# r-papso/carca-replication

Measured on AMD Instinct MI355X. Metric: scored users/sec (1+100 candidates), CARCA eval forward, higher is better.
Workload: dtype f32

## Files before the change

carca_replication_amd/_lib.py:

```python
from __future__ import annotations

import ctypes as C
import hashlib
import os
import shutil
import subprocess
import threading

_HERE = os.path.dirname(os.path.abspath(__file__))
_CSRC = os.path.join(_HERE, "csrc")
_INCLUDE = os.path.join(os.path.dirname(_HERE), "include")
LIB_PATH = os.path.join(_HERE, "libcarca_hip.so")
_STAMP = LIB_PATH + ".srchash"
SOURCES = ["api.hip", "gemm.hip", "gemm_wgrad.hip", "gemm_split.hip", "gemm_stream.hip", "wgrad_cu.hip", "decoders.hip", "batch_build.hip", "embed.hip", "sa_block.hip", "sa_eval.hip", "cross_score.hip", "cross_stream.hip", "loss_metrics.hip", "backward.hip", "block_bwd.hip", "row_chain.hip", "optim.hip", "recommend.hip", "rank.hip", "knn_catalogue.hip",
           "catalogue_xent.hip", "feat_dedup.hip", "sampled_xent.hip", "sampled_bce.hip", "similar_items.hip", "mmr_rerank.hip", "recommend_lists.hip", "explain_lists.hip"]
HEADERS = ["carca_common.h", "gemm_host.h", "attn_common.h", "gemm_epilogue.h", "cross_fold.h", "recommend_common.h", "catalogue_select.h",
           "catalogue_sweep.h", "xent_tile.h", "xent_stage.h", "row_stream.h", "group_select.h"]

MAX_SEGS = 4
MAX_GROUPS = 3
MAX_L = 64
MAX_PROFILE_L = 1024

_lock = threading.Lock()
# ... 299 lines not shown
    "carca_poll_errors": (_i, []),
    "carca_capture_scope": (_i, [_fp, C.POINTER(C.c_ulonglong)]),
    "carca_capture_bytes": (C.c_longlong, [C.c_ulonglong]),
    "carca_capture_release": (_i, [C.c_ulonglong]),
    "carca_release_stream_scratch": (_i, [_fp]),
    "carca_padded_dims": (_i, [_i, _i, C.POINTER(_i), C.POINTER(_i), C.POINTER(_i)]),
    "carca_attn_geometry_built": (_i, [_i, _i]),
    "carca_pack_weights": (_i, [C.POINTER(PackDesc), _i, _fp]),
    "carca_embed_fwd": (_i, [C.POINTER(RowSeg), _i, _i, _i, _i, _i, _fp, _fp, _fp, _fp, _fp, _fp, _fp, _i, _i, _fp]),
    "carca_gemm_rows": (_i, [C.POINTER(GemmDesc), _fp]),
    "carca_split_bytes": (C.c_longlong, [_i, _i, _i]),
    "carca_split_pack": (_i, [_fp, _i, _i, _i, _i, _fp, _fp]),
    "carca_split_bind": (_i, [_fp, _fp, _i, _i, _i]),
    "carca_split_launch_count": (C.c_longlong, []),
    "carca_gemm_rows_group": (_i, [C.POINTER(GemmDesc), _i, _fp]),
    "carca_gemm_wgrad": (_i, [C.POINTER(WgradDesc), _fp]),
    "carca_gemm_wgrad_group": (_i, [C.POINTER(WgradDesc), _i, _fp]),
    "carca_sa_block_fwd": (_i, [_fp, _i, _fp, _fp, _i, _i, _i, _i, _i, C.POINTER(SaWeights), _i, C.POINTER(SaSave),
                                C.POINTER(Dropout), _fp]),
    "carca_sa_block_eval": (_i, [_fp, _i, _fp, _fp, _i, _i, _i, _i, _i, C.POINTER(SaWeights), _i, _i, _fp]),
    "carca_cross_score_fwd": (_i, [_fp, _i, _fp, _fp, C.POINTER(TargetGroup), _i, _i, _i, _i, _i, _i,
                                   C.POINTER(CaWeights), _i, _i, C.POINTER(CaSave), C.POINTER(Dropout), _fp]),
    "carca_dropout_fwd": (_i, [_fp, _i, _i, _i, C.POINTER(Dropout), _fp, _fp]),
    "carca_mask_mul": (_i, [_fp, _i, _fp, _i, _f, _fp, _i, _i, _i, _i, _fp]),
    "carca_layernorm_bwd": (_i, [_fp, _i, _fp, _i, _fp, _i, _i, _fp, _i, _fp, _i, _i, _fp, _fp, _fp]),
    "carca_embed_scatter": (_i, [_fp, _i, _fp, _i, _i, _f, _fp, _fp]),
    "carca_colsum": (_i, [_fp, _i, _i, _i, _fp, _fp, _i, _fp, _fp]),
    "carca_sa_attn_bwd": (_i, [_fp, _fp, _fp, _fp, _i, _fp, _fp, _fp, _fp, _i, _i, _i, _i, _fp, _f, _fp]),
    "carca_cross_attn_bwd": (_i, [_fp, _fp, _fp, C.POINTER(CrossBwdGroup), _i, _fp, _fp, _fp, _fp, _i, _i, _i, _i, _i,
                                  _f, _fp]),
    "carca_unpack_grads": (_i, [C.POINTER(PackDesc), _i, _i, _fp]),
    "carca_forward": (_i, [C.POINTER(ForwardDesc), C.POINTER(_fp), _fp]),
    "carca_event_create": (_i, [C.POINTER(_fp)]),
    "carca_event_destroy": (_i, [_fp]),
    "carca_event_elapsed_ms": (_i, [_fp, _fp, C.POINTER(C.c_float)]),
    "carca_stream_wait_event": (_i, [_fp, _fp]),
    "carca_bce_fwd": (_i, [_fp, _fp, _fp, _i, _f, _fp, _fp, _fp, _fp, _fp]),
    "carca_rank_metrics": (_i, [_fp, _i, _i, _i, _fp, _fp, _fp, _fp]),
    "carca_eval_metrics": (_i, [_fp, _fp, _fp, _i, _i, _i, _f, _fp, _fp]),
    "carca_layernorm_fwd": (_i, [_fp, _i, _fp, _i, _i, _i, _fp, _fp, _fp]),
    "carca_dot_score_fwd": (_i, [_fp, _i, _fp, _i, _fp, _i, _i, _i, _i, _i, _i, _fp]),
    "carca_dot_score_bwd": (_i, [_fp, _i, _fp, _i, _fp, _fp, _fp, _i, _fp, _i, _i, _i, _i, _i, _i, _i, _fp]),
    "carca_slot_decay_scale": (_i, [_fp, _i, _fp, _i, _i, _i, _i, _f, _fp]),
    "carca_l2norm_fwd": (_i, [_fp, _i, _fp, _i, _i, _i, _fp]),
    "carca_l2norm_bwd": (_i, [_fp, _i, _fp, _i, _fp, _i, _i, _i, _fp]),
    "carca_add_positions": (_i, [_fp, _i, _fp, _fp, _i, _i, _i, _i, _fp]),
    "carca_mha_core": (_i, [_fp, _i, _fp, _fp, _i, _fp, _fp, _i, _i, _i, _i, _i, _i, _i, _fp, _i, _fp, _fp]),
    "carca_mha_core_bwd": (_i, [_fp, _i, _fp, _fp, _i, _fp, _fp, _i, _i, _i, _i, _i, _i, _i, _fp, _i, _fp, _fp, _fp, _fp,
                                _fp]),
    "carca_gemm_rows_log": (_i, [C.c_char_p, _i]),
    "carca_feat_dedup_rows_multiplied": (C.c_longlong, []),
    "carca_feat_dedup_rows_computed": (C.c_longlong, []),
    "carca_feat_dedup_rows_grouped": (C.c_longlong, []),
    "carca_feat_cache_arm": (_i, [C.POINTER(FeatCache)]),
    "carca_get_tuning": (_i, [_i]),
    "carca_mha_core_drop": (_i, [_fp, _i, _fp, _fp, _i, _fp, _fp, _i, _i, _i, _i, _i, _i, _i, _fp, _i, _fp, C.POINTER(Dropout),
                                 _fp, _fp]),
    "carca_mha_core_bwd_drop": (_i, [_fp, _i, _fp, _fp, _i, _fp, _fp, _i, _i, _i, _i, _i, _i, _i, _fp, _i, _fp, _fp, _fp, _fp,
                                     _fp, C.c_float, _fp]),
    "carca_knn_score": (_i, [_fp, C.c_int64, _fp, C.c_int64, _fp, _fp, _i, _fp, _i, _i, _i, _i, _fp]),
    "carca_sa_block_bwd_workspace": (C.c_size_t, [_i, _i, _i, _i]),
    "carca_sa_block_bwd": (_i, [C.POINTER(SaBwdDesc), C.POINTER(WgradDesc), C.POINTER(_i), _fp]),
    "carca_cross_score_bwd_workspace": (C.c_size_t, [_i, _i, _i, _i, C.POINTER(C.c_int32), _i]),
    "carca_cross_score_bwd": (_i, [C.POINTER(CrossBwdDesc), C.POINTER(WgradDesc), C.POINTER(_i), _fp]),
    "carca_embed_bwd_workspace": (C.c_size_t, [C.POINTER(C.c_int32), _i, _i, _i]),
    "carca_embed_bwd": (_i, [C.POINTER(EmbedBwdDesc), _fp]),
    "carca_early_event_recorded": (_i, []),
    "carca_adam_step": (_i, [C.POINTER(AdamTensor), _i, C.c_double, C.c_double, C.c_double, C.c_double, C.c_double, _i,
                        _fp]),
    "carca_adam_step_ex": (_i, [C.POINTER(AdamTensor), _i, C.c_double, C.c_double, C.c_double, C.c_double, C.c_double, _i,
                           _i, _fp, _fp]),
    "carca_grad_norm": (_i, [C.POINTER(AdamTensor), _i, C.c_double, _fp, C.c_int64, _fp, _fp]),
    "carca_mark_rows": (_i, [_fp, C.c_int64, _fp, C.c_int64, _fp]),
    "carca_zero_rows": (_i, [_fp, C.c_int64, _i, C.POINTER(_fp), C.POINTER(C.c_int64), _i, _fp]),
    "carca_concat_ids": (_i, [C.POINTER(_fp), C.POINTER(C.c_int64), _i, _fp, _fp]),
    "carca_build_eval_batch": (_i, [_fp, _fp, _fp, _fp, _i, _i, _i, _i, _i, _i, _i, _i, C.c_uint64, _fp, _fp, _fp, _fp, _fp,
                                    _fp]),
    "carca_recommend": (_i, [C.POINTER(RecommendDesc), _fp]),
    "carca_rank_items": (_i, [C.POINTER(RankDesc), _fp]),
    "carca_recommend_among": (_i, [C.POINTER(RecommendDesc), C.POINTER(Candidates), _fp]),
    "carca_rank_items_among": (_i, [C.POINTER(RankDesc), C.POINTER(Candidates), _fp]),
    "carca_recommend_groups": (_i, [C.POINTER(RecommendDesc), C.POINTER(ItemGroups), _fp]),
    "carca_recommend_capped": (_i, [C.POINTER(RecommendDesc), C.POINTER(ItemGroups), _i, _fp]),
    "carca_score_lists": (_i, [C.POINTER(ListsDesc), _fp]),
    "carca_recommend_lists": (_i, [C.POINTER(ListsDesc), _fp]),
    "carca_explain_lists": (_i, [C.POINTER(ExplainDesc), _fp]),
    "carca_knn_recommend": (_i, [C.POINTER(KnnRecommendDesc), _fp]),
    "carca_knn_rank_items": (_i, [C.POINTER(KnnRankDesc), _fp]),
    "carca_row_rnorm": (_i, [_fp, _i, _i, _i, _fp, _fp]),
    "carca_similar_items": (_i, [C.POINTER(SimilarDesc), C.POINTER(Candidates), _fp]),
    "carca_mmr_rerank": (_i, [C.POINTER(MmrDesc), _fp]),
    "carca_catalogue_xent_fwd": (_i, [C.POINTER(CatalogueXentDesc), _fp]),
    "carca_catalogue_xent_bwd": (_i, [C.POINTER(CatalogueXentDesc), _fp]),
    "carca_sampled_xent_fwd": (_i, [C.POINTER(SampledXentDesc), _fp]),
    "carca_sampled_xent_bwd": (_i, [C.POINTER(SampledXentDesc), _fp]),
    "carca_sampled_bce_fwd": (_i, [C.POINTER(SampledBceDesc), _fp]),
    "carca_sampled_bce_bwd": (_i, [C.POINTER(SampledBceDesc), _fp]),
    "carca_build_train_batch": (_i, [_fp, _fp, _fp, _fp, _i, _i, _i, _i, _i, _i, _i, C.c_uint64, _fp, _fp, _fp, _fp, _fp,
                                     _fp]),
}


def declared_symbols() -> list[str]:
    import re

    with open(os.path.join(_INCLUDE, "carca_hip.h")) as f:
# ... 37 lines not shown
```

carca_replication_amd/csrc/carca_common.h:

```cpp
#pragma once
#include <hip/hip_runtime.h>
#include <stdint.h>

#include "../../include/carca_hip.h"

typedef float f32x4 __attribute__((ext_vector_type(4)));
typedef float f32x16 __attribute__((ext_vector_type(16)));
typedef float f32x4_u __attribute__((ext_vector_type(4), aligned(4)));

#define CARCA_WAVE 64

typedef unsigned u32x4 __attribute__((ext_vector_type(4)));
__device__ __forceinline__ __amdgpu_buffer_rsrc_t carca_rsrc(const void* base) {
  return __builtin_amdgcn_make_buffer_rsrc(const_cast<void*>(base), 0, -1, 0x00020000);
}
__device__ __forceinline__ f32x4 gload4(const float* base, int elem_off) {
  const u32x4 v = __builtin_amdgcn_raw_buffer_load_b128(carca_rsrc(base), elem_off * 4, 0, 0);
  f32x4 f = {__uint_as_float(v[0]), __uint_as_float(v[1]), __uint_as_float(v[2]), __uint_as_float(v[3])};
  return f;
}
__device__ __forceinline__ f32x4 gload4s(const float* base, int lane_elem_off, int uniform_elem_off) {
  const u32x4 v = __builtin_amdgcn_raw_buffer_load_b128(carca_rsrc(base), lane_elem_off * 4, uniform_elem_off * 4, 0);
  f32x4 f = {__uint_as_float(v[0]), __uint_as_float(v[1]), __uint_as_float(v[2]), __uint_as_float(v[3])};
  return f;
// ... 111 lines not shown
  float scale;
};
template <int RIF = 1>
__device__ __forceinline__ void carca_gather_rows(const CarcaGatherArgs& ga, int wave, int nwaves, int lane) {
  for (int row0 = wave * RIF; row0 < ga.total_rows; row0 += nwaves * RIF) {
    const float* src[RIF];
#pragma unroll
    for (int i = 0; i < RIF; ++i) {
      const int row = min(row0 + i, ga.total_rows - 1);
      int s = 0;
#pragma unroll
      for (int j = 1; j < 4; ++j)
        if (j < ga.nseg && row >= ga.row_start[j]) s = j;
      src[i] = ga.items_w + (size_t)ga.ids[s][row - ga.row_start[s]] * ga.d;
    }
    for (int c0 = 0; c0 < ga.d; c0 += 64) {
      const int c = c0 + lane;
      float v[RIF];
#pragma unroll
      for (int i = 0; i < RIF; ++i) v[i] = c < ga.d ? src[i][c] : 0.f;
#pragma unroll
      for (int i = 0; i < RIF; ++i)
        if (c < ga.d && row0 + i < ga.total_rows) ga.zq[(size_t)(row0 + i) * ga.ldz + c] = v[i] * ga.scale;
    }
  }
}

template <int BYTES>
__device__ __forceinline__ void carca_warm_kernargs() {
  typedef const __attribute__((address_space(4))) int* karg_ptr;
  karg_ptr ka = (karg_ptr)__builtin_amdgcn_kernarg_segment_ptr();
  int w = 0;
#pragma unroll
  for (int i = 0; i < (BYTES + 63) / 64; ++i) w ^= ka[i * 16];
  asm volatile("" ::"s"(w));
}

enum { CARCA_TUNE_GEMM_VARIANT = 0, CARCA_TUNE_ATTN_VARIANT = 1, CARCA_TUNE_WGRAD_SLOTS = 2,
       CARCA_TUNE_WGRAD_PLAIN_STORE = 3,
       CARCA_TUNE_WGRAD_MIN_CHUNKS = 4,
       CARCA_TUNE_WGRAD_GROUP_SLOTS = 5,
       CARCA_TUNE_N96S_DIAG = 5,
       CARCA_TUNE_ROUND1_PATHS = 6,
       CARCA_TUNE_SCORE_LAYOUT = 7,
       CARCA_TUNE_DETERMINISTIC = 8,
       CARCA_TUNE_STAMPS = 9, CARCA_TUNE_CU_CAP = 10, CARCA_TUNE_SK_DON = 11, CARCA_TUNE_SK_SPIN_LOG2 = 12,
       CARCA_TUNE_SK_WITHHOLD = 13, CARCA_TUNE_XS_OPT = 14, CARCA_TUNE_DIAG = 15, CARCA_TUNE_SPLIT_GEMM = 16,
       CARCA_TUNE_SKC_OV_TEAM = 17,
       CARCA_TUNE_SKC_OV_LONE = 18,
       CARCA_TUNE_SKC_MIN_STEPS = 19,
       CARCA_TUNE_FEAT_DEDUP = 20,
       CARCA_TUNE_FEAT_CACHE = 21,
       CARCA_TUNE_DEDUP_SOLO = 22,
       CARCA_TUNE_COUNT = 24 };
enum {
  CARCA_GV_AUTO = 0,
  CARCA_GV_TILED = 1,
  CARCA_GV_PER_CU = 2,
  CARCA_GV_PER_CU_STAMPS = 3,
  CARCA_GV_NO_BUFFER_LOADS = 4,
  CARCA_GV_WGRAD_TILED = 5,
  CARCA_GV_NO_GROUP = 6,
  CARCA_GV_PER_CU_128 = 7,
  CARCA_GV_NO_PASSENGER = 8,
  CARCA_GV_WIDE64 = 9,
  CARCA_GV_WIDE64_PF2 = 10,
  CARCA_GV_N96 = 11,
  CARCA_GV_NO_N96 = 12,
  CARCA_GV_WGRAD_EQUAL_ITEMS = 13,
  CARCA_GV_WGRAD_ATOMIC_FLUSH = 14,
  CARCA_GV_NO_STREAM_K = 15,
  CARCA_GV_WGRAD_FLAT_GROUPS = 16,
  CARCA_GV_GATHER_ROW_PER_WAVE = 18,
  CARCA_GV_OWN_GATHER = 19,
  CARCA_GV_WPART_ATOMICS = 19,
  CARCA_GV_SPLIT_NO_DMA = 21,
  CARCA_GV_WGRAD_NO_COMPACT = 22,
  CARCA_GV_SK_EVERY_ROW = 23,
  CARCA_GV_NO_CUS = 24,
  CARCA_GV_CUS = 25,
  CARCA_GV_NO_N96S = 26,
  CARCA_GV_N96S = 27,
  CARCA_GV_NO_STREAM_K_NO_PASSENGER = 158,
};
int carca_tuning(int key);
int carca_num_cus();
bool carca_stream_capturing(hipStream_t stream);
void* carca_stream_scratch(hipStream_t stream, int tag, size_t bytes, size_t zero_bytes = 0, bool* fresh = nullptr);
enum { CARCA_SCRATCH_SK = 1, CARCA_SCRATCH_WPART = 2, CARCA_SCRATCH_WTAB = 3, CARCA_SCRATCH_SPLITW = 4, CARCA_SCRATCH_SKC = 5,
       CARCA_SCRATCH_SKC_PART = 6, CARCA_SCRATCH_RECOMMEND = 7, CARCA_SCRATCH_RANK = 8,
       CARCA_SCRATCH_KNN = 9, CARCA_SCRATCH_DEDUP_HASH = 10, CARCA_SCRATCH_DEDUP = 11, CARCA_SCRATCH_SIMILAR = 12,
       CARCA_SCRATCH_LISTS = 13, CARCA_SCRATCH_GROUPS = 14 };
void* carca_capture_alloc(hipStream_t stream, size_t bytes, bool host_mapped, void** device_view, size_t zero_bytes = 0);
void carca_arm_launch_events(void* start, void* stop);
bool carca_take_launch_events(hipEvent_t* start, hipEvent_t* stop);
bool carca_take_feat_cache(CarcaFeatCache* out);
struct CarcaGemmDesc;
void carca_rows_log(const char* kernel, const CarcaGemmDesc* d, int grid);
int carca_gemm_rows_split_try(const CarcaGemmDesc* desc, hipStream_t stream);
int carca_gemm_rows_stream_try(const CarcaGemmDesc* desc, bool fits32, hipStream_t stream);
int carca_gemm_rows_n96s_try(const CarcaGemmDesc* desc, bool fits32, hipStream_t stream);
int carca_gemm_rows_passenger(const CarcaGemmDesc* desc, const CarcaGatherArgs* ga, int* rode, void* stream);
struct CarcaDedupRun {
  CarcaGemmDesc d;
  int nseg, R, vec, vec2, hbits;
  int row0[CARCA_MAX_SEGS + 1];
// ... 53 lines not shown
```

carca_replication_amd/csrc/sa_eval.hip:

```cpp
#include <hip/hip_ext.h>
#include "attn_common.h"
#include "gemm_host.h"
#include "../../include/carca_hip.h"

namespace {

#define SAE_NEG (-1.0e30f)

struct SaEvalArgs {
  const float* x;
  const int32_t* ids;
  float* y;
  int ldx, ldy, L, d, residual, nparts, pads_uniform;
  CarcaSaWeights w;
  float qscale;
  unsigned long long* stamps;
};

template <int DPI, int NCH, bool ISV>
__device__ __forceinline__ void sae_kv_chains(const f32x4 (&wf)[DPI / 16], f32x4 bias4, float bias1, const float* xs, int si,
                                              float* Ks, int so, float* Vt, int ft, int lane) {
  const int ln = lane & 15, mq = lane >> 4;
  const float* x0 = xs + ln * si + 4 * mq;
  f32x4 acc[NCH];
#pragma unroll
  for (int c = 0; c < NCH; ++c) acc[c] = ISV ? f32x4{bias1, bias1, bias1, bias1} : bias4;
#pragma unroll
  for (int kg = 0; kg < DPI / 16; ++kg) {
    f32x4 x[NCH];
#pragma unroll
    for (int c = 0; c < NCH; ++c) x[c] = lds4(x0 + 16 * c * si + 16 * kg);
#pragma unroll
    for (int s = 0; s < 4; ++s)
#pragma unroll
      for (int c = 0; c < NCH; ++c) acc[c] = ISV ? mfma16(x[c][s], wf[kg][s], acc[c]) : mfma16(wf[kg][s], x[c][s], acc[c]);
  }
#pragma unroll
  for (int c = 0; c < NCH; ++c) {
    if (ISV) *reinterpret_cast<f32x4*>(Vt + (16 * ft + ln) * ATT_SK + 16 * c + 4 * mq) = acc[c];
    else *reinterpret_cast<f32x4*>(Ks + (16 * c + ln) * so + 16 * ft + 4 * mq) = acc[c];
  }
}

template <int DPI, int DHP, int NH>
__global__ __launch_bounds__(1024) void sa_eval_kernel(const SaEvalArgs a) {
  using G = AttGeom<DPI, DHP, NH>;
  static_assert(G::SO >= G::SI, "H1 reuses the K image");
  constexpr int NW = 16;
#define SAE_STAMP(i)                                                                                 \
  do {                                                                                               \
    if (a.stamps && threadIdx.x == 0) a.stamps[blockIdx.x * 16 + (i)] = __builtin_readcyclecounter(); \
  } while (0)
  SAE_STAMP(0);
  extern __shared__ __attribute__((aligned(16))) float lds[];
  float* Xs = lds;
  float* Qn = Xs + ATT_LMAX * G::SI;
  float* Ks = Qn + ATT_LMAX * G::SI;
  float* Vt = Ks + ATT_LMAX * G::SO;
  float* Km = Vt + G::DPO * ATT_SK;

  const int L = a.L, d = a.d, nparts = a.nparts;
  const int u = blockIdx.x / nparts, part = blockIdx.x - u * nparts;
  const int tid = threadIdx.x, lane = tid & 63;
  const int wave = __builtin_amdgcn_readfirstlane(tid >> 6);
  const int ln = lane & 15, mq = lane >> 4;
  const size_t ubase = (size_t)u * L;
  const int dh = d / NH;

  const int32_t my_id = gload1i(a.ids + ubase, lane < L ? lane : L - 1);
  constexpr int PPW = (ATT_LMAX / 2) / NW;
  const int half = lane >> 5, c4 = lane & 31;
  const bool col_ok = 4 * c4 < DPI;
  const float* x_user = a.x + ubase * a.ldx;
  f32x4 rv[PPW];
#pragma unroll
  for (int j = 0; j < PPW; ++j) {
    const int r = 2 * (wave + NW * j) + half;
    rv[j] = zero4();
    if (2 * (wave + NW * j) < L) rv[j] = gload4(x_user, (r < L ? r : 0) * a.ldx + (col_ok ? 4 * c4 : 0));
  }
  const f32x4 ln1w = gload4(a.w.ln1_w, col_ok ? 4 * c4 : 0), ln1b = gload4(a.w.ln1_b, col_ok ? 4 * c4 : 0);
  constexpr int NBJ = 2 * G::NF;
  f32x4 bwf[G::NKG], bb4;
  float bb1;
  if (wave < NBJ) {
    const int j = wave;
    const bool isv = j >= G::NF;
    const int ft = isv ? j - G::NF : j;
    const float* wp = isv ? a.w.wv : a.w.wk;
#pragma unroll
    for (int kg = 0; kg < G::NKG; ++kg) bwf[kg] = gload4s(wp, 4 * lane, 256 * (ft * G::NKG + kg));
    bb4 = gload4s(a.w.bk, 4 * mq, 16 * ft);
    bb1 = gload1(a.w.bv, 16 * ft + ln);
  }
  const unsigned long long pmask = __ballot(lane < L && my_id != 0);
  const int s0 = a.pads_uniform ? (pmask ? (int)__builtin_ctzll(pmask) : L) : 0;
  const int nk = L - s0;
  const int rep = s0 > 0 ? 1 : 0;
  const int nrows = nk + rep;
  const int LT = (nrows + 15) >> 4;
  const unsigned tmask = nparts == 1 ? (1u << LT) - 1u
                         : LT == 4   ? (part == 0 ? 0x6u : 0x9u)
                         : LT == 3   ? (part == 0 ? 0x4u : 0x3u)
                         : LT == 2   ? (part == 0 ? 0x2u : 0x1u)
                                     : (part == 0 ? 0x1u : 0x0u);
  if (tmask == 0) return;
  unsigned own_packed = 0;
  int n_own = 0, kmax = 0;
#pragma unroll
  for (int t = 0; t < ATT_LT; ++t)
    if (t < LT && ((tmask >> t) & 1u)) {
      own_packed |= (unsigned)t << (4 * n_own);
      ++n_own;
      kmax = t + 1;
    }
  auto own = [&](int i) { return (int)((own_packed >> (4 * i)) & 15u); };
  SAE_STAMP(1);

  {
    const float inv_d = 1.0f / (float)d;
#pragma unroll
    for (int j = 0; j < PPW; ++j) {
      const int r = 2 * (wave + NW * j) + half;
      const int t = r >= s0 ? r - s0 : (r == 0 ? nk : -1);
      const bool keep = r < L && t >= 0;
      f32x4 v = rv[j];
#pragma unroll
      for (int e = 0; e < 4; ++e) v[e] = (4 * c4 + e < d) ? v[e] : 0.f;
      const float mean = half32_sum((v[0] + v[1]) + (v[2] + v[3])) * inv_d;
      f32x4 dv, q;
#pragma unroll
      for (int e = 0; e < 4; ++e) dv[e] = (4 * c4 + e < d) ? v[e] - mean : 0.f;
      const float var = half32_sum((dv[0] * dv[0] + dv[1] * dv[1]) + (dv[2] * dv[2] + dv[3] * dv[3])) * inv_d;
      const float rstd = 1.0f / sqrtf(var + 1e-5f);
#pragma unroll
      for (int e = 0; e < 4; ++e) q[e] = (4 * c4 + e < d) ? dv[e] * rstd * ln1w[e] + ln1b[e] : 0.f;
      if (keep && col_ok) {
        *reinterpret_cast<f32x4*>(Xs + t * G::SI + 4 * c4) = v;
        *reinterpret_cast<f32x4*>(Qn + t * G::SI + 4 * c4) = q;
      }
    }
    for (int t = nrows + 2 * wave + half; t < 16 * LT; t += 2 * NW)
      if (col_ok) {
        *reinterpret_cast<f32x4*>(Xs + t * G::SI + 4 * c4) = zero4();
        *reinterpret_cast<f32x4*>(Qn + t * G::SI + 4 * c4) = zero4();
      }
    if (wave == NW - 1) Km[lane] = (lane < nk && ((pmask >> (lane + s0)) & 1ull)) ? 0.f : SAE_NEG;
    __syncthreads();
  }
  SAE_STAMP(2);
  {
    bool first = true;
    for (int job = wave; job < NBJ; job += NW) {
      const bool isv = job >= G::NF;
      const int ft = isv ? job - G::NF : job;
      if (!first) {
        const float* wp = isv ? a.w.wv : a.w.wk;
#pragma unroll
        for (int kg = 0; kg < G::NKG; ++kg) bwf[kg] = gload4s(wp, 4 * lane, 256 * (ft * G::NKG + kg));
        bb4 = gload4s(a.w.bk, 4 * mq, 16 * ft);
        bb1 = gload1(a.w.bv, 16 * ft + ln);
      }
      first = false;
      if (isv) {
        if (kmax > 3) sae_kv_chains<DPI, 4, true>(bwf, bb4, bb1, Xs, G::SI, Ks, G::SO, Vt, ft, lane);
        else if (kmax > 2) sae_kv_chains<DPI, 3, true>(bwf, bb4, bb1, Xs, G::SI, Ks, G::SO, Vt, ft, lane);
        else sae_kv_chains<DPI, 2, true>(bwf, bb4, bb1, Xs, G::SI, Ks, G::SO, Vt, ft, lane);
      } else {
        if (kmax > 3) sae_kv_chains<DPI, 4, false>(bwf, bb4, bb1, Xs, G::SI, Ks, G::SO, Vt, ft, lane);
        else if (kmax > 2) sae_kv_chains<DPI, 3, false>(bwf, bb4, bb1, Xs, G::SI, Ks, G::SO, Vt, ft, lane);
        else sae_kv_chains<DPI, 2, false>(bwf, bb4, bb1, Xs, G::SI, Ks, G::SO, Vt, ft, lane);
      }
    }
  }
  __syncthreads();
  SAE_STAMP(3);

  for (int job = wave; job < n_own * NH; job += NW) {
    const int qi = job / NH, h = job - qi * NH;
    const int qt = own(qi);
    const int q = 16 * qt + ln;
    f32x4 qfrag[G::NKG];
#pragma unroll
    for (int kg = 0; kg < G::NKG; ++kg) qfrag[kg] = lds4(Qn + q * G::SI + 16 * kg + 4 * mq);
    f32x4 qh[G::NFH];
#pragma unroll
    for (int ft = 0; ft < G::NFH; ++ft) {
      f32x4 wf[G::NKG];
#pragma unroll
      for (int kg = 0; kg < G::NKG; ++kg) wf[kg] = gload4s(a.w.wq, 4 * lane, 256 * ((h * G::NFH + ft) * G::NKG + kg));
      const f32x4 bias = gload4s(a.w.bq, 4 * mq, h * DHP + 16 * ft);
      CARCA_PIN_LOADS();
      f32x4 acc = zero4();
#pragma unroll
      for (int kg = 0; kg < G::NKG; ++kg) acc = mfma16_group(wf[kg], qfrag[kg], acc);
      qh[ft] = (acc + bias) * a.qscale;
    }
    f32x4 sc[ATT_LT];
    float mx = SAE_NEG;
#pragma unroll
    for (int kt = 0; kt < ATT_LT; ++kt) {
      if (kt <= qt) {
        f32x4 acc = lds4(Km + 16 * kt + 4 * mq);
        if (kt == qt) {
#pragma unroll
          for (int r = 0; r < 4; ++r) acc[r] = (4 * mq + r <= ln) ? acc[r] : SAE_NEG;
        }
        const float* krow = Ks + (16 * kt + ln) * G::SO + h * DHP + 4 * mq;
#pragma unroll
        for (int ft = 0; ft < G::NFH; ++ft) acc = mfma16_group(lds4(krow + 16 * ft), qh[ft], acc);
        sc[kt] = acc;
        mx = fmaxf(fmaxf(mx, fmaxf(acc[0], acc[1])), fmaxf(acc[2], acc[3]));
      }
    }
    mx = quad4_max(mx);
    const bool q_ok = Km[q] == 0.f;
    float sum = 0.f;
#pragma unroll
    for (int kt = 0; kt < ATT_LT; ++kt) {
      if (kt <= qt) {
#pragma unroll
        for (int r = 0; r < 4; ++r) {
          const float e = __builtin_amdgcn_exp2f(sc[kt][r] - mx);
          sc[kt][r] = e;
          sum += e;
        }
      }
    }
// ... 32 lines not shown
      for (int e = 0; e < 4; ++e) dv[e] = (4 * c4 + e < d) ? v[e] - mean : 0.f;
      const float var = half32_sum((dv[0] * dv[0] + dv[1] * dv[1]) + (dv[2] * dv[2] + dv[3] * dv[3])) * inv_d;
      const float rstd = 1.0f / sqrtf(var + 1e-5f);
#pragma unroll
      for (int e = 0; e < 4; ++e) v[e] = (4 * c4 + e < d) ? dv[e] * rstd * ln2w[e] + ln2b[e] : 0.f;
      if (col_ok) *reinterpret_cast<f32x4*>(Xs + r * G::SI + 4 * c4) = v;
    }
  }
  __syncthreads();
  SAE_STAMP(5);
  float* H1 = Ks;
  for (int job = wave; job < n_own * G::NKG; job += NW) {
    const int qi = job / G::NKG, ft = job - qi * G::NKG;
    const int q = 16 * own(qi) + ln;
    const float* srow = Xs + q * G::SI + 4 * mq;
    f32x4 wf[G::NKG];
#pragma unroll
    for (int kg = 0; kg < G::NKG; ++kg) wf[kg] = gload4s(a.w.w1, 4 * lane, 256 * (ft * G::NKG + kg));
    f32x4 acc = gload4s(a.w.b1, 4 * mq, 16 * ft);
    CARCA_PIN_LOADS();
#pragma unroll
    for (int kg = 0; kg < G::NKG; ++kg) acc = mfma16_group(wf[kg], lds4(srow + 16 * kg), acc);
#pragma unroll
    for (int r = 0; r < 4; ++r) acc[r] = acc[r] > 0.f ? acc[r] : 0.01f * acc[r];
    *reinterpret_cast<f32x4*>(H1 + q * G::SI + 16 * ft + 4 * mq) = acc;
  }
  __syncthreads();
  SAE_STAMP(6);
  for (int job = wave; job < n_own * G::NKG; job += NW) {
    const int qi = job / G::NKG, ft = job - qi * G::NKG;
    const int q = 16 * own(qi) + ln;
    const float* hrow = H1 + q * G::SI + 4 * mq;
    f32x4 wf[G::NKG];
#pragma unroll
    for (int kg = 0; kg < G::NKG; ++kg) wf[kg] = gload4s(a.w.w2, 4 * lane, 256 * (ft * G::NKG + kg));
    f32x4 acc = gload4s(a.w.b2, 4 * mq, 16 * ft);
    CARCA_PIN_LOADS();
#pragma unroll
    for (int kg = 0; kg < G::NKG; ++kg) acc = mfma16_group(wf[kg], lds4(hrow + 16 * kg), acc);
    if (a.residual) acc = acc + lds4(Xs + q * G::SI + 16 * ft + 4 * mq);
    if (16 * ft + 4 * mq < a.ldy) {
      float* yu = a.y + ubase * a.ldy + 16 * ft + 4 * mq;
      if (q < nk) {
        *reinterpret_cast<f32x4*>(yu + (size_t)(q + s0) * a.ldy) = acc;
      } else if (q == nk && rep) {
        for (int j = 0; j < s0; ++j) *reinterpret_cast<f32x4*>(yu + (size_t)j * a.ldy) = acc;
      }
    }
  }
  SAE_STAMP(7);
#undef SAE_STAMP
}

template <int DPI, int DHP, int NH>
int launch_sa_eval(SaEvalArgs& a, int B, hipStream_t stream) {
  using G = AttGeom<DPI, DHP, NH>;
  const size_t lds_bytes = sizeof(float) * (2 * ATT_LMAX * G::SI + ATT_LMAX * G::SO + G::DPO * ATT_SK + ATT_LMAX);
  auto kern = sa_eval_kernel<DPI, DHP, NH>;
  static bool attr_set = false;
  if (!attr_set) {
    hipError_t e = hipFuncSetAttribute((const void*)kern, hipFuncAttributeMaxDynamicSharedMemorySize, (int)lds_bytes);
    if (e != hipSuccess) {
      carca_set_error("sa_block_fwd: cannot reserve %zu B of LDS: %s", lds_bytes, hipGetErrorString(e));
      return (int)e;
    }
    attr_set = true;
  }
  const int tune = carca_tuning(CARCA_TUNE_ATTN_VARIANT);
  a.nparts = (a.L > 16 && tune != 1 && (tune == 2 || 2 * B <= carca_num_cus())) ? 2 : 1;
  carca_launch(kern, dim3(B * a.nparts), dim3(1024), lds_bytes, stream, true, a);
  CARCA_LAUNCH_CHECK();
  return CARCA_OK;
}

}

int carca_sa_eval_launch(const float* x, int ldx, const int32_t* ids, float* y, int ldy, int B, int L, int d, int H,
                         const CarcaSaWeights* w, int residual, int pads_uniform, hipStream_t stream) {
  int dpi, dhp, dpo;
  if (carca_padded_dims(d, H, &dpi, &dhp, &dpo) != CARCA_OK) return CARCA_ERR_UNSUPPORTED;
  SaEvalArgs a{};
  a.x = x; a.ids = ids; a.y = y; a.ldx = ldx; a.ldy = ldy; a.L = L; a.d = d; a.residual = residual;
  a.pads_uniform = pads_uniform;
  a.w = *w;
  a.qscale = (float)(1.4426950408889634 / sqrt((double)(d / H)));
  a.stamps = carca_debug_buffer();
  CARCA_ATT_DISPATCH(launch_sa_eval, a, B, stream);
  carca_set_error("sa_block_fwd: no kernel built for d=%d H=%d (padded %d / head %d)", d, H, dpi, dhp);
  return CARCA_ERR_UNSUPPORTED;
}
```

carca_replication_amd/ops.py:

```python
from __future__ import annotations

import ctypes as C
import functools
import math
from dataclasses import dataclass
from typing import Iterable, List, Optional, Sequence, Tuple

import torch
from torch import Tensor

from . import _lib
from ._lib import CarcaHipError


_stage_events = None


def set_stage_events(ev) -> None:
    global _stage_events
    _stage_events = ev


_fused_events = None

# ... 1081 lines not shown

def num_cus() -> int:
    return torch.cuda.get_device_properties(torch.cuda.current_device()).multi_processor_count


def poll_errors() -> None:
    _lib.check(_lib.load().carca_poll_errors(), "poll_errors")


def capture_scope() -> int:
    out = C.c_ulonglong(0)
    _lib.check(_lib.load().carca_capture_scope(_stream(), C.byref(out)), "capture_scope")
    return int(out.value)


def capture_bytes(scope: int) -> int:
    return int(_lib.load().carca_capture_bytes(C.c_ulonglong(scope)))


def capture_release(scope: int) -> None:
    if scope:
        _lib.check(_lib.load().carca_capture_release(C.c_ulonglong(scope)), "capture_release")


TUNE_SPLIT_GEMM = 16
SPLIT_GEMM_MODES = {"fp32": 0, "bf16x3": 1, "fp16x2": 2}
_split_mode = 0


def gemm_rows_log(on: Optional[bool] = None) -> str:
    lib = _lib.load()
    if on is not None:
        lib.carca_gemm_rows_log(None, int(bool(on)))
        return ""
    buf = C.create_string_buffer(65536)
    lib.carca_gemm_rows_log(buf, len(buf))
    return buf.value.decode()


def feat_dedup_rows_multiplied() -> int:
    return int(_lib.load().carca_feat_dedup_rows_multiplied())


def feat_dedup_rows_computed() -> int:
    return int(_lib.load().carca_feat_dedup_rows_computed())


def feat_dedup_rows_grouped() -> int:
    return int(_lib.load().carca_feat_dedup_rows_grouped())


TUNE_FEAT_CACHE = 21
TUNE_DEDUP_SOLO = 22


def get_tuning(key: int) -> int:
    return int(_lib.load().carca_get_tuning(int(key)))


def set_feature_gemm_precision(mode: str, force: bool = False) -> None:
    global _split_mode
    set_tuning(TUNE_SPLIT_GEMM, SPLIT_GEMM_MODES[mode] | (16 if force and SPLIT_GEMM_MODES[mode] else 0))
    _split_mode = SPLIT_GEMM_MODES[mode]
    if _split_mode == 0:
        _lib.check(_lib.load().carca_split_bind(None, None, 0, 0, 0), "split_bind")


def feature_gemm_mode() -> int:
    return _split_mode


def split_launch_count() -> int:
    return int(_lib.load().carca_split_launch_count())


def split_pack(w: Tensor, K0: int, mode: int) -> Tensor:
    w = _f32(w.detach())
    _need_cuda(w)
    lib = _lib.load()
    N = w.shape[0]
    out = torch.empty(int(lib.carca_split_bytes(N, int(K0), int(mode))), dtype=torch.uint8, device=w.device)
    _lib.check(lib.carca_split_pack(w.data_ptr(), w.stride(0), int(K0), N, int(mode), out.data_ptr(), _stream()), "split_pack")
    return out


def split_bind(w: Optional[Tensor], planes: Optional[Tensor], mode: int = 0, K0: int = 0) -> None:
    lib = _lib.load()
    if w is None:
        _lib.check(lib.carca_split_bind(None, None, 0, 0, 0), "split_bind")
    else:
        _lib.check(lib.carca_split_bind(w.data_ptr(), planes.data_ptr(), int(mode), w.shape[0], int(K0)), "split_bind")


CX_TILE = 64
CX_MAX_SPLITS = 256
CX_WAVES_PER_CU = 4


def _xent_plan(R: int, n_classes: int, d: int, n_cus: int, extra_dp_partials: int,
               share_partials: bool = False) -> Tuple[int, int, int, int, int]:
    r64 = lambda n: (n + 63) // 64 * 64
    ldo = (d + 3) // 4 * 4
    target = CX_WAVES_PER_CU * max(1, int(n_cus))
    n_row_blocks = -(-R // CX_TILE)
    n_class_blocks = -(-n_classes // CX_TILE)
    s_c = max(1, min(n_class_blocks, CX_MAX_SPLITS, -(-target // n_row_blocks)))
# ... 339 lines not shown
```

include/carca_hip.h:

```cpp
#ifndef CARCA_HIP_H
#define CARCA_HIP_H

#include <stdint.h>

#ifdef __cplusplus
extern "C" {
#endif

#define CARCA_ABI_VERSION 3
#define CARCA_OK 0
#define CARCA_ERR_UNSUPPORTED (-1)
#define CARCA_ERR_BADARG (-2)

#define CARCA_MAX_SEGS 4
#define CARCA_MAX_GROUPS 3
#define CARCA_MAX_L 64
#define CARCA_MAX_PROFILE_L 1024
#define CARCA_EMBED_GATHER 1
#define CARCA_EMBED_FEAT 2
#define CARCA_EMBED_JOINT 4
#define CARCA_EMBED_ALL 7
#define CARCA_EMBED_DEDUP 8

int carca_abi_version(void);
// ... 85 lines not shown
  int32_t mask_rows;
} CarcaWgradDesc;
int carca_gemm_wgrad(const CarcaWgradDesc* desc , void* stream);
int carca_gemm_wgrad_group(const CarcaWgradDesc* descs , int n, void* stream);

typedef struct CarcaRowSeg {
  const int32_t* ids;
  const float* attrs;
  const float* ctx;
  float* e_out;
  int32_t rows;
  int32_t T;
  int32_t add_pos;
  int64_t attrs_bstride, ctx_bstride;
  const float* attrs_table;
  int32_t attrs_table_rows;
} CarcaRowSeg;
int carca_embed_fwd(const CarcaRowSeg* segs , int nseg, int n_attrs, int n_ctx, int d, int g,
                    const float* items_w , const float* feats_w ,
                    const float* feats_b , const float* joint_w , const float* joint_b ,
                    const float* pos , float* zq, int ld_e, int stages, void* stream);

typedef struct CarcaSaWeights {
  const float *ln1_w, *ln1_b, *ln2_w, *ln2_b;
  const float *wq, *wk, *wv;
  const float *bq, *bk, *bv;
  const float *w1, *w2;
  const float *b1, *b2;
} CarcaSaWeights;
typedef struct CarcaDropout {
  float p;
  uint64_t seed;
  uint32_t site;
  const uint64_t* seed_offset;
} CarcaDropout;

typedef struct CarcaSaSave {
  float* qn;
  float *qh, *kh, *vh;
  float* r;
  float* s2;
  float* h1;
  uint8_t* m_attn;
  uint8_t* m_ffn1;
  uint8_t* m_ffn2;
} CarcaSaSave;
int carca_sa_block_fwd(const float* x , int ldx, const int32_t* ids , float* y ,
                       int ldy, int B, int L, int d, int H, const CarcaSaWeights* w , int residual,
                       const CarcaSaSave* save , const CarcaDropout* drop ,
                       void* stream);

int carca_sa_block_eval(const float* x, int ldx, const int32_t* ids, float* y, int ldy, int B, int L, int d, int H,
                        const CarcaSaWeights* w , int residual, int pads_uniform, void* stream);

typedef struct CarcaCaWeights {
  const float *ln_w, *ln_b;
  const float *wq, *wk, *wv;
  const float *bq, *bk, *bv;
  const float* ffn_w_pad;
  const float* ffn_w;
  const float* ffn_b;
  const float *wu, *cu;
} CarcaCaWeights;
typedef struct CarcaTargetGroup {
  const float* o;
  const int32_t* ids;
  float* y;
  int32_t N;
  int32_t ldy;
} CarcaTargetGroup;
typedef struct CarcaCaSave {
  float *kh, *vh;
  float* qh[CARCA_MAX_GROUPS];
  uint8_t* m_attn[CARCA_MAX_GROUPS];
} CarcaCaSave;
int carca_cross_score_fwd(const float* p_raw , int ldp,
                          const int32_t* p_ids , float* p_normed ,
                          const CarcaTargetGroup* groups , int ngroups, int ldo, int B, int L, int d, int H,
                          const CarcaCaWeights* w , int residual, int training,
                          const CarcaCaSave* save , const CarcaDropout* drop ,
                          void* stream);

int carca_layernorm_bwd(const float* dy, int ld_dy, const float* x, int ld_x, const float* gamma, int rows, int d,
                        const float* addend , int ld_add, float* dx, int ld_dx, int ncols_out,
                        float* dgamma , float* dbeta , void* stream);
int carca_embed_scatter(const float* dz, int ld_dz, const int32_t* ids, int rows, int d, float scale,
                        float* d_items , void* stream);
int carca_colsum(const float* x, int ld_x, int rows, int cols, const float* rowscale, const int32_t* ids, int T,
                 float* out , void* stream);
int carca_sa_attn_bwd(const float* qh, const float* kh, const float* vh, const float* d_attn, int ld_da,
                      const int32_t* ids, float* dqh, float* dkh, float* dvh, int B, int L, int d, int H,
                      const uint8_t* m_attn , float drop_scale , void* stream);
typedef struct CarcaCrossBwdGroup {
  const float* qh;
  const float* y;
  const float* dy;
  const int32_t* ids;
  float* dqh;
  float* dlogit;
  const uint8_t* m_attn;
  int32_t N;
  int32_t ld_y;
} CarcaCrossBwdGroup;
int carca_cross_attn_bwd(const float* kh, const float* vh, const int32_t* p_ids, const CarcaCrossBwdGroup* groups,
                         int ngroups, const float* ffn_w_pad, float* dkh, float* dvh, float* d_ffn_w_pad, int B, int L,
                         int d, int H, int training, float drop_scale, void* stream);
// ... 510 lines not shown
```

Measured before the change: 773,200.

## Lend idle SA-eval blocks to heavy users via in-kernel work plan

In the two-part self-attention eval kernel, blocks whose user has too few non-pad rows to own any query tile now build a per-batch plan in LDS from every user's ids. They then take over query tiles of users that need all four tiles, so work is spread more evenly across blocks. Heavy users' blocks read the same plan and shrink their own tile mask to match. This adds a small id scan and ballot logic per block, plus a debug counter readable from the host. It only applies when pads are uniform, L>48 and B<=128.

```diff
diff --git a/carca_replication_amd/_lib.py b/carca_replication_amd/_lib.py
--- a/carca_replication_amd/_lib.py
+++ b/carca_replication_amd/_lib.py
@@ -375,6 +375,7 @@
     "carca_feat_dedup_rows_multiplied": (C.c_longlong, []),
     "carca_feat_dedup_rows_computed": (C.c_longlong, []),
     "carca_feat_dedup_rows_grouped": (C.c_longlong, []),
+    "carca_sa_eval_lent": (C.c_longlong, []),
     "carca_feat_cache_arm": (_i, [C.POINTER(FeatCache)]),
     "carca_get_tuning": (_i, [_i]),
     "carca_mha_core_drop": (_i, [_fp, _i, _fp, _fp, _i, _fp, _fp, _i, _i, _i, _i, _i, _i, _i, _fp, _i, _fp, C.POINTER(Dropout),
diff --git a/carca_replication_amd/csrc/carca_common.h b/carca_replication_amd/csrc/carca_common.h
--- a/carca_replication_amd/csrc/carca_common.h
+++ b/carca_replication_amd/csrc/carca_common.h
@@ -187,6 +187,7 @@
        CARCA_TUNE_FEAT_DEDUP = 20,
        CARCA_TUNE_FEAT_CACHE = 21,
        CARCA_TUNE_DEDUP_SOLO = 22,
+       CARCA_TUNE_SA_LEND = 23,
        CARCA_TUNE_COUNT = 24 };
 enum {
   CARCA_GV_AUTO = 0,
diff --git a/carca_replication_amd/csrc/sa_eval.hip b/carca_replication_amd/csrc/sa_eval.hip
--- a/carca_replication_amd/csrc/sa_eval.hip
+++ b/carca_replication_amd/csrc/sa_eval.hip
@@ -15,7 +15,47 @@
   CarcaSaWeights w;
   float qscale;
   unsigned long long* stamps;
+  int lend;
+  int count;
 };
+
+__device__ unsigned sae_lent_word;
+
+#define SAE_PLAN_USERS 128
+
+__device__ __forceinline__ u32x4 gload4i(const int32_t* base, int elem_off) {
+  return __builtin_amdgcn_raw_buffer_load_b128(carca_rsrc(base), elem_off * 4, 0, 0);
+}
+
+struct SaePlan {
+  unsigned long long d_lo, d_hi, r_lo, r_hi;
+  int t_lo, t_hi;
+  __device__ __forceinline__ static int below(unsigned long long lo, unsigned long long hi, int u) {
+    return u < 64 ? __popcll(lo & ((1ull << u) - 1ull)) : __popcll(lo) + __popcll(hi & ((1ull << (u - 64)) - 1ull));
+  }
+  __device__ __forceinline__ int donors() const { return __popcll(d_lo) + __popcll(d_hi); }
+  __device__ __forceinline__ int recipients() const { return __popcll(r_lo) + __popcll(r_hi); }
+  __device__ __forceinline__ int lent() const { return min(donors(), 2 * recipients()); }
+  __device__ __forceinline__ int share(int r) const { return max(0, min(2, donors() - 2 * r)); }
+  __device__ __forceinline__ int donor_rank(int u) const { return below(d_lo, d_hi, u); }
+  __device__ __forceinline__ int recipient_rank(int u) const { return below(r_lo, r_hi, u); }
+  __device__ __forceinline__ int recipient(int r, int lane) const {
+    const unsigned long long lt = (1ull << lane) - 1ull;
+    const unsigned long long s_lo = __ballot(t_lo == 4 && __popcll(r_lo & lt) == r);
+    const unsigned long long s_hi = __ballot(t_hi == 4 && __popcll(r_lo) + __popcll(r_hi & lt) == r);
+    return s_lo ? (int)__builtin_ctzll(s_lo) : 64 + (int)__builtin_ctzll(s_hi | (1ull << 63));
+  }
+};
+__device__ __forceinline__ SaePlan sae_read_plan(const unsigned char* LTs, int lane) {
+  SaePlan p;
+  p.t_lo = LTs[lane];
+  p.t_hi = LTs[lane + 64];
+  p.d_lo = __ballot(p.t_lo == 1);
+  p.d_hi = __ballot(p.t_hi == 1);
+  p.r_lo = __ballot(p.t_lo == 4);
+  p.r_hi = __ballot(p.t_hi == 4);
+  return p;
+}
 
 template <int DPI, int NCH, bool ISV>
 __device__ __forceinline__ void sae_kv_chains(const f32x4 (&wf)[DPI / 16], f32x4 bias4, float bias1, const float* xs, int si,
@@ -60,25 +100,30 @@
   float* Km = Vt + G::DPO * ATT_SK;
 
   const int L = a.L, d = a.d, nparts = a.nparts;
-  const int u = blockIdx.x / nparts, part = blockIdx.x - u * nparts;
+  int u = blockIdx.x / nparts;
+  const int part = blockIdx.x - u * nparts;
   const int tid = threadIdx.x, lane = tid & 63;
   const int wave = __builtin_amdgcn_readfirstlane(tid >> 6);
   const int ln = lane & 15, mq = lane >> 4;
-  const size_t ubase = (size_t)u * L;
+  size_t ubase = (size_t)u * L;
   const int dh = d / NH;
-
-  const int32_t my_id = gload1i(a.ids + ubase, lane < L ? lane : L - 1);
+  unsigned char* LTs = reinterpret_cast<unsigned char*>(Km + ATT_LMAX);
+
+  int32_t my_id = gload1i(a.ids + ubase, lane < L ? lane : L - 1);
   constexpr int PPW = (ATT_LMAX / 2) / NW;
   const int half = lane >> 5, c4 = lane & 31;
   const bool col_ok = 4 * c4 < DPI;
   const float* x_user = a.x + ubase * a.ldx;
   f32x4 rv[PPW];
-#pragma unroll
-  for (int j = 0; j < PPW; ++j) {
-    const int r = 2 * (wave + NW * j) + half;
-    rv[j] = zero4();
-    if (2 * (wave + NW * j) < L) rv[j] = gload4(x_user, (r < L ? r : 0) * a.ldx + (col_ok ? 4 * c4 : 0));
-  }
+  auto request_rows = [&]() {
+#pragma unroll
+    for (int j = 0; j < PPW; ++j) {
+      const int r = 2 * (wave + NW * j) + half;
+      rv[j] = zero4();
+      if (2 * (wave + NW * j) < L) rv[j] = gload4(x_user, (r < L ? r : 0) * a.ldx + (col_ok ? 4 * c4 : 0));
+    }
+  };
+  request_rows();
   const f32x4 ln1w = gload4(a.w.ln1_w, col_ok ? 4 * c4 : 0), ln1b = gload4(a.w.ln1_b, col_ok ? 4 * c4 : 0);
   constexpr int NBJ = 2 * G::NF;
   f32x4 bwf[G::NKG], bb4;
@@ -93,28 +138,68 @@
     bb4 = gload4s(a.w.bk, 4 * mq, 16 * ft);
     bb1 = gload1(a.w.bv, 16 * ft + ln);
   }
-  const unsigned long long pmask = __ballot(lane < L && my_id != 0);
-  const int s0 = a.pads_uniform ? (pmask ? (int)__builtin_ctzll(pmask) : L) : 0;
-  const int nk = L - s0;
-  const int rep = s0 > 0 ? 1 : 0;
-  const int nrows = nk + rep;
-  const int LT = (nrows + 15) >> 4;
-  const unsigned tmask = nparts == 1 ? (1u << LT) - 1u
-                         : LT == 4   ? (part == 0 ? 0x6u : 0x9u)
-                         : LT == 3   ? (part == 0 ? 0x4u : 0x3u)
-                         : LT == 2   ? (part == 0 ? 0x2u : 0x1u)
-                                     : (part == 0 ? 0x1u : 0x0u);
-  if (tmask == 0) return;
-  unsigned own_packed = 0;
-  int n_own = 0, kmax = 0;
-#pragma unroll
-  for (int t = 0; t < ATT_LT; ++t)
-    if (t < LT && ((tmask >> t) & 1u)) {
-      own_packed |= (unsigned)t << (4 * n_own);
-      ++n_own;
-      kmax = t + 1;
-    }
-  auto own = [&](int i) { return (int)((own_packed >> (4 * i)) & 15u); };
+  unsigned long long pmask = __ballot(lane < L && my_id != 0);
+  int s0 = a.pads_uniform ? (pmask ? (int)__builtin_ctzll(pmask) : L) : 0;
+  int nk = L - s0;
+  int rep = s0 > 0 ? 1 : 0;
+  int nrows = nk + rep;
+  int LT = (nrows + 15) >> 4;
+  unsigned tmask = nparts == 1 ? (1u << LT) - 1u
+                   : LT == 4   ? (part == 0 ? 0x6u : 0x9u)
+                   : LT == 3   ? (part == 0 ? 0x4u : 0x3u)
+                   : LT == 2   ? (part == 0 ? 0x2u : 0x1u)
+                               : (part == 0 ? 0x1u : 0x0u);
+  const int nusers = gridDim.x / nparts;
+  const bool reporter = a.lend && a.count && blockIdx.x == 1;
+  const bool planner = a.lend && (tmask == 0 || LT == 4 || blockIdx.x == 1);
+  u32x4 pv[2];
+  auto request_plan = [&]() {
+    const int ps = L - 4 * (ln + 1) > 0 ? L - 4 * (ln + 1) : 0;
+#pragma unroll
+    for (int i = 0; i < 2; ++i) {
+      const int pu = 4 * (NW * i + wave) + mq;
+      pv[i] = gload4i(a.ids, (pu < nusers ? pu : 0) * L + ps);
+    }
+  };
+  auto plan_to_lds = [&]() {
+    const int ps = L - 4 * (ln + 1) > 0 ? L - 4 * (ln + 1) : 0;
+#pragma unroll
+    for (int i = 0; i < 2; ++i) {
+      const int pu = 4 * (NW * i + wave) + mq;
+      int f = ATT_LMAX;
+#pragma unroll
+      for (int e = 3; e >= 0; --e) f = pv[i][e] != 0u ? ps + e : f;
+      if (L - 4 * ln <= 0) f = ATT_LMAX;
+      const int first = ATT_LMAX - (int)row16_max((float)(ATT_LMAX - f));
+      const int ps0 = first < L ? first : L;
+      const int prow = L - ps0 + (ps0 > 0 ? 1 : 0);
+      if (ln == 0) LTs[pu] = pu < nusers ? (unsigned char)((prow + 15) >> 4) : (unsigned char)0;
+    }
+  };
+  bool donor = false;
+  if (tmask == 0) {
+    if (!a.lend) return;
+    request_plan();
+    plan_to_lds();
+    __syncthreads();
+    const SaePlan p = sae_read_plan(LTs, lane);
+    if (reporter && tid == 0) sae_lent_word = (unsigned)p.lent();
+    const int k = p.donor_rank(u), r = k >> 1;
+    if (r >= p.recipients()) return;
+    tmask = p.share(r) == 2 ? ((k & 1) ? 0x1u : 0x2u) : 0x3u;
+    donor = true;
+    u = min(__builtin_amdgcn_readfirstlane(p.recipient(r, lane)), nusers - 1);
+    ubase = (size_t)u * L;
+    x_user = a.x + ubase * a.ldx;
+    my_id = gload1i(a.ids + ubase, lane < L ? lane : L - 1);
+    request_rows();
+    pmask = __ballot(lane < L && my_id != 0);
+    s0 = pmask ? (int)__builtin_ctzll(pmask) : L;
+    nk = L - s0;
+    rep = s0 > 0 ? 1 : 0;
+    nrows = nk + rep;
+    LT = (nrows + 15) >> 4;
+  }
   SAE_STAMP(1);
 
   {
@@ -149,6 +234,8 @@
     __syncthreads();
   }
   SAE_STAMP(2);
+  if (planner && !donor) request_plan();
+  const int kmax = min(LT, 32 - (int)__builtin_clz(tmask));
   {
     bool first = true;
     for (int job = wave; job < NBJ; job += NW) {
@@ -173,7 +260,23 @@
       }
     }
   }
+  if (planner && !donor) plan_to_lds();
   __syncthreads();
+  if (planner && !donor) {
+    const SaePlan p = sae_read_plan(LTs, lane);
+    if (LT == 4 && p.share(p.recipient_rank(u)) > 0) tmask = part == 0 ? 0x4u : 0x8u;
+    if (reporter && tid == 0) sae_lent_word = (unsigned)p.lent();
+  }
+  if (!a.lend && a.count && blockIdx.x == 0 && tid == 0) sae_lent_word = 0u;
+  unsigned own_packed = 0;
+  int n_own = 0;
+#pragma unroll
+  for (int t = 0; t < ATT_LT; ++t)
+    if (t < LT && ((tmask >> t) & 1u)) {
+      own_packed |= (unsigned)t << (4 * n_own);
+      ++n_own;
+    }
+  auto own = [&](int i) { return (int)((own_packed >> (4 * i)) & 15u); };
   SAE_STAMP(3);
 
   for (int job = wave; job < n_own * NH; job += NW) {
@@ -312,10 +415,17 @@
 #undef SAE_STAMP
 }
 
+struct SaeLast {
+  hipStream_t stream;
+  bool valid;
+};
+thread_local SaeLast g_sae_last{nullptr, false};
+
 template <int DPI, int DHP, int NH>
 int launch_sa_eval(SaEvalArgs& a, int B, hipStream_t stream) {
   using G = AttGeom<DPI, DHP, NH>;
-  const size_t lds_bytes = sizeof(float) * (2 * ATT_LMAX * G::SI + ATT_LMAX * G::SO + G::DPO * ATT_SK + ATT_LMAX);
+  const size_t lds_bytes =
+      sizeof(float) * (2 * ATT_LMAX * G::SI + ATT_LMAX * G::SO + G::DPO * ATT_SK + ATT_LMAX) + SAE_PLAN_USERS;
   auto kern = sa_eval_kernel<DPI, DHP, NH>;
   static bool attr_set = false;
   if (!attr_set) {
@@ -328,11 +438,27 @@
   }
   const int tune = carca_tuning(CARCA_TUNE_ATTN_VARIANT);
   a.nparts = (a.L > 16 && tune != 1 && (tune == 2 || 2 * B <= carca_num_cus())) ? 2 : 1;
+  a.lend = (a.nparts == 2 && a.pads_uniform && a.L > 3 * 16 && B <= SAE_PLAN_USERS && carca_tuning(CARCA_TUNE_SA_LEND) != 1) ? 1 : 0;
+  const bool cap = carca_stream_capturing(stream);
+  a.count = cap ? 0 : 1;
   carca_launch(kern, dim3(B * a.nparts), dim3(1024), lds_bytes, stream, true, a);
   CARCA_LAUNCH_CHECK();
+  if (!cap) g_sae_last = SaeLast{stream, true};
   return CARCA_OK;
 }
 
+}
+
+extern "C" long long carca_sa_eval_lent(void) {
+  const SaeLast l = g_sae_last;
+  if (!l.valid) return -1;
+  void* word = nullptr;
+  unsigned n = 0;
+  if (hipGetSymbolAddress(&word, HIP_SYMBOL(sae_lent_word)) != hipSuccess ||
+      hipMemcpyAsync(&n, word, sizeof(n), hipMemcpyDeviceToHost, l.stream) != hipSuccess ||
+      hipStreamSynchronize(l.stream) != hipSuccess)
+    return -1;
+  return (long long)n;
 }
 
 int carca_sa_eval_launch(const float* x, int ldx, const int32_t* ids, float* y, int ldy, int B, int L, int d, int H,
diff --git a/carca_replication_amd/ops.py b/carca_replication_amd/ops.py
--- a/carca_replication_amd/ops.py
+++ b/carca_replication_amd/ops.py
@@ -1157,6 +1157,11 @@
 
 TUNE_FEAT_CACHE = 21
 TUNE_DEDUP_SOLO = 22
+TUNE_SA_LEND = 23
+
+
+def sa_eval_lent() -> int:
+    return int(_lib.load().carca_sa_eval_lent())
 
 
 def get_tuning(key: int) -> int:
diff --git a/include/carca_hip.h b/include/carca_hip.h
--- a/include/carca_hip.h
+++ b/include/carca_hip.h
@@ -161,6 +161,7 @@
 
 int carca_sa_block_eval(const float* x, int ldx, const int32_t* ids, float* y, int ldy, int B, int L, int d, int H,
                         const CarcaSaWeights* w , int residual, int pads_uniform, void* stream);
+long long carca_sa_eval_lent(void);
 
 typedef struct CarcaCaWeights {
   const float *ln_w, *ln_b;
```

Result: faster. 783,200, median of 6 (+1.3%).
